# ygtxr1997/MSML

Measured on AMD Instinct MI355X. Metric: images/sec (112x112) ires50-MSML+PartialFC training step, higher is better.
Workload: dtype bf16; 1 GPU; iresnet50-MSML (OSB r18 + FM x4) + 85742-id ArcFace PartialFC, 112x112, batch 256/GPU, fwd+bwd+clip+SGD; global_batch=256, parallelism=dp1+class-parallel head, launch=eager, weight gradients + OSB on side streams

## Files before the change

include/msml_hip.h:

```cpp
#ifndef MSML_HIP_H
#define MSML_HIP_H

#include <stddef.h>
#include <stdint.h>

#ifdef __cplusplus
extern "C" {
#endif

#define MSML_ABI_VERSION 1

enum { MSML_F32 = 0, MSML_BF16 = 1, MSML_BF16X3 = 2 };

enum {
  MSML_OK = 0,
  MSML_ERR_SHAPE = -1,
  MSML_ERR_DTYPE = -2,
  MSML_ERR_LAUNCH = -3,
  MSML_ERR_UNSUPPORTED = -4,
  MSML_ERR_WORKSPACE = -5
};

enum { MSML_ACT_TANH = 0, MSML_ACT_SIGMOID = 1 };
enum { MSML_ARITH_ADD = 0, MSML_ARITH_SUB = 1, MSML_ARITH_MUL = 2, MSML_ARITH_DIV = 3 };
// ... 60 lines not shown
int msml_bn_stats_rows(long M, int C);
int msml_bn_stats(const void* x, long M, int C, float* partial, int dtype, void* stream);
int msml_bn_finalize(const float* partial, int rows, int C, double count, const float* gamma,
                     const float* beta, float* running_mean, float* running_var, float momentum,
                     float eps, float* scale, float* shift, float* save_mean, float* save_invstd,
                     void* stream);
int msml_bn_act_fwd(const void* x, const float* scale, const float* shift, const float* alpha,
                    const void* residual, int res_first, void* y, long M, int C, int dtype,
                    void* stream);
int msml_bn_act_fwd_stats_rows(long M, int C);
int msml_bn_act_fwd_stats(const void* x, const float* scale, const float* shift, const float* alpha,
                          const void* residual, int res_first, void* y, long M, int C,
                          float* stats, int dtype, void* stream);
int msml_bn_fin_act_fwd(const double* acc, double count, const float* gamma, const float* beta,
                        float* running_mean, float* running_var, float momentum, float eps, float* scale,
                        float* shift, float* save_mean, float* save_invstd, const void* x,
                        const float* alpha, const void* residual, int res_first, void* y, long M, int C,
                        double* acc_out, int dtype, void* stream);
int msml_bn_stats_acc(const void* x, long M, int C, double* acc, int dtype, void* stream);
int msml_conv2d_bnbwd_acc(const void* in0, int c0p, const void* wp, int kop, void* out, int coutp, int N,
                          int H, int W, int P, int Q, int R, int S, int stride, int pad_h, int pad_w,
                          int transposed, const void* bn_x, const float* bn_scale, const float* bn_shift,
                          const float* bn_alpha, const float* bn_mean, const float* bn_invstd, double* acc,
                          void* stream);
int msml_bn_fin_bwd_apply(const void* dy, const void* x, const float* scale, const float* shift,
                          const float* alpha, const float* save_mean, const float* save_invstd,
                          const double* acc, const void* residual_first, const void* add, int add_h,
                          int add_w, void* dx, void* dres, float* dgamma, float* dbeta, float* dalpha,
                          int accumulate, long M, int C, const void* next_x, const float* next_mean,
                          const float* next_invstd, double* next_acc, int dtype, void* stream);
int msml_bn_act_bwd_acc(const void* dy, const void* x, const float* scale, const float* shift,
                        const float* alpha, const float* save_mean, const float* save_invstd,
                        const void* residual_first, const void* add, void* dx, void* dres, float* dgamma,
                        float* dbeta, float* dalpha, int accumulate, long M, int C, double* acc, int dtype,
                        void* stream);
int msml_bn_act_bwd(const void* dy, const void* x, const float* scale, const float* shift,
                    const float* alpha, const float* save_mean, const float* save_invstd,
                    const void* residual_first, void* dx, void* dres, float* dgamma, float* dbeta,
                    float* dalpha, int accumulate, long M, int C, float* workspace, long ws_floats,
                    int dtype, void* stream);
int msml_bias_grad(const void* dy, long M, int Cp, int Creal, float* db, int accumulate,
                   float* workspace, long ws_floats, int dtype, void* stream);
int msml_add(const void* a, const void* b, void* out, long n, int dtype, void* stream);

int msml_dap_fwd(const void* x, float* seg, unsigned char* mask, int N, int H, int W, int Cp,
                 int dtype, void* stream);
int msml_dap_bwd(const float* dseg, void* dx, int N, int H, int W, int Cp, int dtype, void* stream);
int msml_seg_consensus_loss(const float* logit, const long* msk, int N, int H, int W, float alpha,
                            float beta, float* loss, float* dlogit, float* workspace,
                            long ws_floats, void* stream);
int msml_seg_consensus_loss_r(const float* logit, const long* msk, int N, int H, int W, float alpha, float beta,
                              int reduce_pixel_all, int reduce_pixel_kl_all, float* loss, float* dlogit,
                              float* workspace, long ws_floats, void* stream);

int msml_rownorm_fwd(const float* w, int R, int Rp, int E, void* dst, int ld, float* inv_norm,
                     int dtype, void* stream);
int msml_rownorm_bwd(const float* w, const float* inv_norm, const float* dy, int ldy, int R, int E,
                     float* dw, int accumulate, void* stream);
int msml_gather_target(const float* cosm, int ld, const long* label, int N, float* out,
                       void* stream);
int msml_margin_fwd(float* cosm, const long* label, int N, int C, int ld, int kind, float s,
                    float m, float a, float k, void* stream);
int msml_margin_bwd(const float* dlogit, int ldg, const long* label, const float* cos_t, int N,
                    int C, void* dcos, int ldo, int kind, float s, float m, float a, float k,
                    int dtype, void* stream);
int msml_pfc_rowstats(const float* cosm, int ld, int N, int C, const long* label, int kind, float s,
                      float m, float a, float k, float* rowmax, float* rowsum, void* stream);
int msml_pfc_grad(const float* cosm, int ld, int N, int C, const long* label, int kind, float s,
                  float m, float a, float k, const float* gmax, const float* gsum, float eps_ls,
                  float inv_n, void* dcos, int ldo, float* ptarget, int dtype, void* stream);
int msml_sgd_momentum(float* w, const float* grad, float* mom, long n, float lr, float mu, float wd,
                      int first_step, const float* clip_coef, void* stream);
int msml_grad_norm_clip(const float* grad, long n, float max_norm, float* out2, float* workspace,
                        long ws_floats, void* stream);
int msml_sgd_momentum_dev(float* w, const float* grad, float* mom, long n, const float* lr, float mu, float wd,
                          const float* coef, void* stream);
int msml_grad_norm_clip_scaled(const float* grad, long n, float max_norm, float scale, float* out2, float* workspace,
                               long ws_floats, void* stream);

long msml_gemm_splitk_workspace(int M, int coutp, int K);
int msml_gemm_splitk(const void* a, int M, int K, const void* wp, int kop, float* out, int coutp,
                     void* workspace, long ws_bytes, int dtype, void* stream);

int msml_pack_weights_batched(const long* table, int count, int dtype, void* stream);
int msml_pack_tiles(int A, int B, int R, int S);
int msml_pack_weights_tiled(const long* table, const int* tile_prefix, int count, int total_tiles,
                            int dtype, void* stream);

int msml_transpose(const void* src, int R, int C, int ld_s, void* dst, int ld_d, int dtype,
                   void* stream);

int msml_conv2d_fused(const void* in0, int c0p, const void* in1, int c1p, const void* wp, int kop,
                      const float* scale, const float* shift, const float* alpha,
                      const void* residual, int res_first, void* out, int coutp, int N, int H,
                      int W, int P, int Q, int R, int S, int stride, int pad_h, int pad_w,
                      int transposed, void* stream);

int msml_conv2d_x3(const void* in0, int c0p, const void* in1, int c1p, const void* wp, int kop,
                   const float* scale, const float* shift, const float* alpha, const void* residual,
                   int res_first, void* out, int coutp, int N, int H, int W, int P, int Q, int R, int S,
                   int stride, int pad_h, int pad_w, int transposed, void* stream);
int msml_conv2d_x3_border(const void* in0, int c0p, const void* wp, int kop, const float* scale,
                          const float* shift9, const float* alpha, const void* residual, int res_first,
                          void* out, int coutp, int N, int H, int W, void* stream);
int msml_x3_bn_act_fwd(const void* x, const float* scale, const float* shift, const float* alpha,
                       const void* residual, int res_first, void* y, long M, int C, void* stream);
int msml_x3_fm_fuse_fwd(const void* x, const void* yf, void* z, long M, int C, int act, int arith,
                        void* stream);
int msml_x3_add(const void* a, const void* b, void* out, long M, int C, void* stream);
int msml_x3_from_f32(const float* src, void* dst, long M, int C, void* stream);
int msml_x3_to_f32(const void* src, float* dst, long M, int C, void* stream);

int msml_pair_sqdist(const float* emb, int n_pairs, int E, double* dist, void* stream);
int msml_pair_sqdist_f64(const double* emb, int n_pairs, int E, double* dist, void* stream);
int msml_pair_hist(const double* dist, const unsigned char* same, int n_pairs, const double* thr, int nthr,
                   int nfolds, int* hist, void* stream);

int msml_occ_draw(long seed, long offset, int N, int H, int W, int mode, int lo, int hi, int flip, int* desc,
                  void* stream);
int msml_occ_apply(const unsigned char* src, const int* desc, float* img, long* msk, float* ori, int N, int H,
                   int W, int light, void* stream);

int msml_occ_draw_tex(long seed, long offset, int N, int H, int W, int mode, int lo, int hi, int flip,
                      const int* meta, int nsets, int* desc, void* stream);
int msml_occ_resize(const unsigned char* atlas, const int* meta, const int* dir, const int* rtab, const int* desc,
                    unsigned char* patch, long patch_stride, int N, int lds_bytes, void* stream);
int msml_occ_apply_tex(const unsigned char* src, const int* desc, const unsigned char* patch, long patch_stride,
                       float* img, long* msk, float* ori, int N, int H, int W, int light, void* stream);

int msml_occ_draw_out(long seed, long offset, int N, int H, int W, int out_h, int out_w, int mode, int lo, int hi,
                      int flip, const int* meta, int nsets, int* desc, void* stream);
int msml_occ_apply_out(const unsigned char* src, const int* desc, const unsigned char* patch, long patch_stride,
                       const int* tabw, const int* tabh, float* img, long* msk, float* ori, int N, int H, int W,
                       int out_h, int out_w, int gray, int norm, int light, void* stream);

int msml_deconv4_bwd_data(const void* dy, const void* wp0, const void* wp1, void* dx0, void* dx1, int N, int H,
                          void* stream);

int msml_conv2d_bnbwd_rows(int coutp, int N, int P, int Q);
int msml_conv2d_bnbwd(const void* in0, int c0p, const void* wp, int kop, void* out, int coutp,
                      int N, int H, int W, int P, int Q, int R, int S, int stride, int pad_h,
                      int pad_w, int transposed, const void* bn_x, const float* bn_scale,
                      const float* bn_shift, const float* bn_alpha, const float* bn_mean,
                      const float* bn_invstd, float* partial, int rows_cap, int* rows_used,
                      void* stream);
int msml_bn_act_bwd_apply(const void* dy, const void* x, const float* scale, const float* shift,
                          const float* alpha, const float* save_mean, const float* save_invstd,
                          const float* partial, int rows, const void* add, void* dx,
                          float* dgamma, float* dbeta, float* dalpha, int accumulate, long M,
                          int C, float* coef_ws, int dtype, void* stream);

int msml_bn_act_bwd_apply_s2(const void* dy, const void* x, const float* scale, const float* shift,
                             const float* alpha, const float* save_mean, const float* save_invstd,
                             const float* partial, int rows, const void* add, int H, int W, void* dx,
                             float* dgamma, float* dbeta, float* dalpha, int accumulate, long M,
                             int C, float* coef_ws, int dtype, void* stream);
int msml_bn_act_bwd_apply_next_s2(const void* dy, const void* x, const float* scale,
                                  const float* shift, const float* alpha, const float* save_mean,
                                  const float* save_invstd, const float* partial, int rows,
                                  const void* add, int H, int W, void* dx, float* dgamma, float* dbeta,
                                  float* dalpha, int accumulate, long M, int C, float* coef_ws,
                                  const void* next_x, const float* next_mean,
                                  const float* next_invstd, float* next_partial, int dtype,
                                  void* stream);

int msml_conv2d_bnin_applies(int c0p, int coutp, int N, int H, int W, int P, int Q, int R, int S,
// ... 80 lines not shown
```

msml_amd/headers/partial_fc.py:

```python
import logging
import os

import torch
import torch.distributed as dist
from torch.nn import Module
from torch.nn.parameter import Parameter


_FORCE = bool(os.environ.get("MSML_FORCE_DIST"))


class _Margin:
    kind = "arc"

    def __init__(self, s=64.0, m=0.5, a=0.0, k=0.0):
        self.s, self.m, self.a, self.k = float(s), float(m), float(a), float(k)

    def __call__(self, logits, labels):
        raise TypeError("msml_amd margins are descriptors consumed by the fused HIP kernels")


class ArcMargin(_Margin):
    kind = "arc"


class CosMargin(_Margin):
    kind = "cos"


class HipBackend:

    def __init__(self, dtype):
        from .. import ops
        from .._lib import TORCH_DTYPE, call
        self.ops, self.call, self.dtype = ops, call, dtype
        self.tdt = TORCH_DTYPE[dtype]

    def local_stats(self, total_features, sub_weight, labels, margin):
        ops, call = self.ops, self.call
        from .. import functional as Fh
        n, e = total_features.shape
        c = sub_weight.shape[0]
        dev = total_features.device
        cp = ops.cpad(c)
        kop = (cp + ops.tile_n(cp) - 1) // ops.tile_n(cp) * ops.tile_n(cp)
        wn = torch.empty(kop, e, dtype=self.tdt, device=dev)
        inv_w = torch.empty(c, dtype=torch.float32, device=dev)
        call("msml_rownorm_fwd", sub_weight.detach(), c, kop, e, wn, e, inv_w, self.dtype)
        xs = total_features.to(self.tdt).reshape(n, 1, 1, e).contiguous()
        cosm, _ = ops.conv2d(xs, None, wn, None, cp, 1, 1, 1, 0, 0, False, out_dtype=0)
        cosm = cosm.reshape(n, cp)
        rowmax = torch.empty(n, dtype=torch.float32, device=dev)
        rowsum = torch.empty(n, dtype=torch.float32, device=dev)
        kind = Fh.HEAD_KIND[margin.kind]
        call("msml_pfc_rowstats", cosm, cp, n, c, labels, kind, margin.s, margin.m, margin.a,
             margin.k, rowmax, rowsum)
        state = (xs, wn, inv_w, cosm, kind)
        return state, rowmax, rowsum

    def local_grads(self, state, sub_weight, labels, margin, gmax, gsum, n_total, eps_ls, dw_out=None):
        ops, call = self.ops, self.call
        xs, wn, inv_w, cosm, kind = state
        n, cp = cosm.shape
        c, e = sub_weight.shape
        dev = cosm.device
        dcos = torch.empty(n, 1, 1, cp, dtype=self.tdt, device=dev)
        ptarget = torch.empty(n, dtype=torch.float32, device=dev)
        call("msml_pfc_grad", cosm, cp, n, c, labels, kind, margin.s, margin.m, margin.a, margin.k,
             gmax, gsum, eps_ls, 1.0 / n_total, dcos, cp, ptarget, self.dtype)
        wnt = torch.empty(e, ops.kpad(cp), dtype=self.tdt, device=dev)
        call("msml_transpose", wn, c, e, e, wnt, ops.kpad(cp), self.dtype)
        if self.dtype == 1:
            dx = ops.gemm_splitk(dcos.reshape(n, cp), wnt, e)
        else:
            dx, _ = ops.conv2d(dcos, None, wnt, None, e, 1, 1, 1, 0, 0, False, out_dtype=0)
        dwn = torch.empty(c, e, dtype=torch.float32, device=dev)
        ops.conv_wgrad(dcos, xs, dwn, c, e, e, 0, 1, 1, 1, 0, 0)
        dw = dw_out if dw_out is not None else torch.empty(c, e, dtype=torch.float32, device=dev)
        call("msml_rownorm_bwd", sub_weight.detach(), inv_w, dwn, e, c, e, dw, 0)
        return ptarget, dx.reshape(n, e), dw


class PartialFC(Module):
    @torch.no_grad()
    def __init__(self, rank, local_rank, world_size, batch_size, resume, margin_softmax, num_classes,
                 sample_rate=1.0, embedding_size=512, prefix="./", fp16=False, backend=None,
                 device=None):
        super().__init__()
        if not isinstance(margin_softmax, _Margin):
            raise TypeError("margin_softmax must be msml_amd.headers.ArcMargin / CosMargin "
                            "(the margin is fused into the HIP softmax kernels)")
        self.num_classes, self.rank, self.local_rank = num_classes, rank, local_rank
        self.device = device if device is not None else torch.device("cuda:{}".format(local_rank))
        self.world_size, self.batch_size = world_size, batch_size
        self.margin_softmax = margin_softmax
        self.sample_rate, self.embedding_size, self.prefix = sample_rate, embedding_size, prefix
        self.num_local = num_classes // world_size + int(rank < num_classes % world_size)
        self.class_start = num_classes // world_size * rank + min(rank, num_classes % world_size)
        self.num_sample = int(self.sample_rate * self.num_local)
        self.weight_name = os.path.join(prefix, "rank:{}_softmax_weight.pt".format(rank))
        self.weight_mom_name = os.path.join(prefix, "rank:{}_softmax_weight_mom.pt".format(rank))
        self.weight = self.weight_mom = None
        if resume:
            try:
                self.weight = torch.load(self.weight_name).to(self.device)
                logging.info("softmax weight resume successfully!")
            except (FileNotFoundError, KeyError, IndexError):
                logging.info("softmax weight resume fail!")
            try:
                self.weight_mom = torch.load(self.weight_mom_name).to(self.device)
                logging.info("softmax weight mom resume successfully!")
            except (FileNotFoundError, KeyError, IndexError):
                logging.info("softmax weight mom resume fail!")
        if self.weight is None:
            self.weight = torch.normal(0, 0.01, (self.num_local, embedding_size), device=self.device)
        if self.weight_mom is None:
            self.weight_mom = torch.zeros_like(self.weight)
        self.stream = torch.cuda.Stream(local_rank) if self.device.type == "cuda" else None
        self.index = None
        self.full = int(self.sample_rate) == 1
        if self.full:
            self.sub_weight = Parameter(self.weight)
            self.sub_weight_mom = self.weight_mom
        else:
            self.sub_weight = Parameter(torch.empty((0, 0), device=self.device))
            self.sub_weight_mom = None
        self._k = None
        self._flat_param = None
        if backend is None:
            from .._lib import BF16, F32
            backend = HipBackend(BF16 if fp16 else F32)
        self.backend = backend
        self.eps_ls = 0.1
        self._stage = None
        self._flat = None
        self._label_job = None
        self.perm_fn = None

    def save_params(self):
        if not self.full and self.index is not None:
            self.update()
        w = self.sub_weight.data if self.full else self.weight
        mom = self.sub_weight_mom if self.full else self.weight_mom
        torch.save(w.detach().clone(), self.weight_name)
        torch.save(mom.detach().clone(), self.weight_mom_name)

    def adopt_flat_optimizer(self, opt):
        if not self.full:
            if self._flat_param is None or self.sub_weight is not self._flat_param or id(self.sub_weight) not in opt.offsets:
                raise ValueError("negative sampling on a flat-arena optimizer: build it over pfc.flat_parameter() "
                                 "(and adopt it before the first prefetch_labels() / forward_backward())")
            if opt.max_norm is not None:
                raise ValueError("the head's FlatSGD must be built with max_norm=None (the reference never clips the "
                                 "PartialFC weight, train.py:267-277)")
            self._flat_mom = opt.momentum_view(self.sub_weight)
            opt.steps = max(opt.steps, 1)
            self._flat = opt
            return
        mview = opt.momentum_view(self.sub_weight)
        mview.copy_(self.weight_mom)
        if self.weight_mom.abs().sum().item() != 0:
            opt.steps = max(opt.steps, 1)
# ... 175 lines not shown
```

msml_amd/csrc/wgrad_halo.hip:

```cpp
#include <stdlib.h>

#include <type_traits>

#include <mutex>

#include "common.h"

typedef __attribute__((ext_vector_type(4))) short s16x4;
typedef __attribute__((ext_vector_type(8))) short s16x8;
typedef __attribute__((address_space(3))) void* lptr_t;

#define WH_OOB 0x78000000u

#define WH_MAXGROUP 8
struct WgradHaloArgs {
  const unsigned short* u[WH_MAXGROUP]; int up; unsigned int u_bytes;
  const unsigned short* v[WH_MAXGROUP]; int vp; unsigned int v_bytes;
  int N, H, W, spy, spx;
  int XH, XW;
  int nstrips, chunk;
  int zper;
  int remap;
  int pair7;
  float* ws;
  BnIn xin;
};

template <int CO, bool XF = false, bool P7 = false>
__global__ void __launch_bounds__(512) __attribute__((amdgpu_waves_per_eu(2, 2))) k_wgrad_halo(const WgradHaloArgs p) {
#if defined(__HIP_DEVICE_COMPILE__)
  constexpr int NXB = 20;
  constexpr int GU = CO / 32, NI = CO / 64, UBLK = 7 * GU, NBLK = UBLK + NXB, NISS = (NBLK + 7) / 8;
  constexpr int UB = UBLK * 1024, VB = NXB * 1024, STAGE = UB + VB;
  extern __shared__ __attribute__((aligned(16))) char smem[];
  MSML_LDS_REGION(smem, 2 * STAGE + (XF ? 3 * 64 * 4 : 0));
  const int t = threadIdx.x, lane = t & 63;
  const int wave = __builtin_amdgcn_readfirstlane(t >> 6);
  const int mp = wave & 1, nh = (wave >> 1) & 1, tg = wave >> 2;
  int bx = blockIdx.x, by = blockIdx.y, bz = blockIdx.z;
  if (p.remap) {
    const int T = gridDim.x * gridDim.y, total = T * gridDim.z;
    const int L = bx + gridDim.x * (by + gridDim.y * bz);
    const int Lp = (L & 7) * (total >> 3) + (L >> 3);
    const int tile = Lp % T;
    bz = Lp / T;
    bx = tile % gridDim.x;
    by = tile / gridDim.x;
  }
  const int layer = __builtin_amdgcn_readfirstlane(bz / p.zper);
  const int a0 = bx * CO, b0 = by * 64, split = bz - layer * p.zper;
  const int s_begin = split * p.chunk;
  int s_end = s_begin + p.chunk;
  if (s_end > p.nstrips) s_end = p.nstrips;
  const int spi = p.spy * p.spx;

  __amdgpu_buffer_rsrc_t rs_u = __builtin_amdgcn_make_buffer_rsrc((void*)p.u[layer], 0, (int)p.u_bytes, 0x00020000);
  __amdgpu_buffer_rsrc_t rs_v = __builtin_amdgcn_make_buffer_rsrc((void*)p.v[layer], 0, (int)p.v_bytes, 0x00020000);

  const int lp = lane >> 2, lc = lane & 3;
  auto issue = [&](int strip, int buf) {
    char* ub = smem + buf * STAGE;
    char* vb = ub + UB;
    if constexpr (P7) {
      const int n = 2 * strip + (lp >> 3), x = lp & 7;
      const bool img = n < p.N;
#pragma unroll
      for (int i = 0; i < NISS; i++) {
        const int blk = wave + 8 * i;
        if (blk >= NBLK) break;
        if (blk < UBLK) {
          const int j = blk / GU, g = blk % GU;
          const unsigned int off = (img & (x < 7)) ? (unsigned int)((n * 7 + j) * 7 + x) * (unsigned int)(p.up * 2) +
                                                         (unsigned int)(a0 + g * 32 + lc * 8) * 2u
                                                   : WH_OOB;
          __builtin_amdgcn_raw_ptr_buffer_load_lds(rs_u, (lptr_t)(ub + blk * 1024), 16, off, 0, 0, 0);
        } else {
          const int bb = blk - UBLK, hr = bb >> 1, g = bb & 1;
          const int y = hr - 1;
          const bool ok = img & ((unsigned)y < 7u) & (x > 0);
          const unsigned int off = ok ? (unsigned int)((n * 7 + y) * 7 + x - 1) * (unsigned int)(p.vp * 2) +
                                            (unsigned int)(b0 + g * 32 + lc * 8) * 2u
                                      : WH_OOB;
          __builtin_amdgcn_raw_ptr_buffer_load_lds(rs_v, (lptr_t)(vb + bb * 1024), 16, off, 0, 0, 0);
        }
      }
      return;
    }
    const int n = strip / spi, rem = strip - n * spi, sy = rem / p.spx;
    const int y0 = sy * 7, x0 = (rem - sy * p.spx) * 14;
#pragma unroll
    for (int i = 0; i < NISS; i++) {
      const int blk = wave + 8 * i;
      if (blk >= NBLK) break;
      if (blk < UBLK) {
        const int j = blk / GU, g = blk % GU;
        const int y = y0 + j, x = x0 + lp;
        const bool ok = (lp < 14) & (x < p.W) & (y < p.H);
        const unsigned int off = ok ? (unsigned int)((n * p.H + y) * p.W + x) * (unsigned int)(p.up * 2) +
                                          (unsigned int)(a0 + g * 32 + lc * 8) * 2u
                                    : WH_OOB;
        __builtin_amdgcn_raw_ptr_buffer_load_lds(rs_u, (lptr_t)(ub + blk * 1024), 16, off, 0, 0, 0);
      } else {
        const int bb = blk - UBLK, hr = bb >> 1, g = bb & 1;
        const int y = y0 + hr - 1, x = x0 + lp - 1;
        const bool ok = (hr < 9) & ((unsigned)y < (unsigned)p.H) & ((unsigned)x < (unsigned)p.W);
        const unsigned int off = ok ? (unsigned int)((n * p.H + y) * p.W + x) * (unsigned int)(p.vp * 2) +
                                          (unsigned int)(b0 + g * 32 + lc * 8) * 2u
                                    : WH_OOB;
        __builtin_amdgcn_raw_ptr_buffer_load_lds(rs_v, (lptr_t)(vb + bb * 1024), 16, off, 0, 0, 0);
      }
    }
  };

  float* xtab = reinterpret_cast<float*>(smem + 2 * STAGE);
  auto xform = [&](int strip, int buf) {
    const int n = strip / spi, rem = strip - n * spi, sy = rem / p.spx;
    const int y0 = sy * 7, x0 = (rem - sy * p.spx) * 14;
    char* vb = smem + buf * STAGE + UB;
    const bool has_alpha = p.xin.alpha != nullptr;
#pragma unroll
    for (int i = 0; i < NISS; i++) {
      const int blk = wave + 8 * i;
      if (blk >= NBLK) break;
      if (blk >= UBLK) {
        const int bb = blk - UBLK, hr = bb >> 1, g = bb & 1;
        const int y = y0 + hr - 1, x = x0 + lp - 1;
        if ((hr < 9) & ((unsigned)y < (unsigned)p.H) & ((unsigned)x < (unsigned)p.W))
          bn_in_chunk(vb + bb * 1024 + lane * 16, xtab, 64, g * 32 + lc * 8, has_alpha);
      }
    }
  };

  f32x16 acc[NI][5];
#pragma unroll
  for (int i = 0; i < NI; i++)
#pragma unroll
    for (int k = 0; k < 5; k++)
#pragma unroll
      for (int e = 0; e < 16; e++) acc[i][k][e] = 0.f;

  const int g4 = lane >> 4, i16 = lane & 15, q4 = i16 >> 2, pp = i16 & 3;
  const int px = 8 * (g4 >> 1) + q4;
  const int chan = (2 * (g4 & 1) + (pp >> 1)) * 16 + (pp & 1) * 8;
  const int aofs = mp * NI * 1024 + px * 64 + chan;
  int vlo[3], vhi[3];
#pragma unroll
  for (int s = 0; s < 3; s++) {
    const int p0 = px + s, p1 = px + 4 + s;
    vlo[s] = nh * 1024 + (p0 >> 4) * 2048 + (p0 & 15) * 64 + chan;
    vhi[s] = nh * 1024 + (p1 >> 4) * 2048 + (p1 & 15) * 64 + chan;
  }
  const int ntaps = tg == 0 ? 5 : 4, tap0 = tg * 5;
  int vlok[5], vhik[5];
#pragma unroll
  for (int k = 0; k < 5; k++) {
    const int tp = tap0 + k, r = tp / 3, sft = tp - r * 3;
    vlok[k] = r * 2048 + (sft == 0 ? vlo[0] : (sft == 1 ? vlo[1] : vlo[2]));
    vhik[k] = r * 2048 + (sft == 0 ? vhi[0] : (sft == 1 ? vhi[1] : vhi[2]));
  }
  typedef __attribute__((address_space(3))) s16x4* tr_ptr;
  auto tr2 = [&](const char* lo, const char* hi) -> s16x8 {
    s16x4 l = __builtin_amdgcn_ds_read_tr16_b64_v4i16((tr_ptr)(lo));
    s16x4 h = __builtin_amdgcn_ds_read_tr16_b64_v4i16((tr_ptr)(hi));
    s16x8 o;
    o[0] = l[0]; o[1] = l[1]; o[2] = l[2]; o[3] = l[3];
    o[4] = h[0]; o[5] = h[1]; o[6] = h[2]; o[7] = h[3];
    return o;
  };

  if (s_begin < s_end) issue(s_begin, 0);
  if (XF) bn_in_fill(p.xin, xtab, b0, 64, t, 512);
  __syncthreads();
  if (XF) {
    if (s_begin < s_end) xform(s_begin, 0);
    __syncthreads();
  }
  int cur = 0;
  s16x8 fa[2][NI], fb5[2][5];
  for (int strip = s_begin; strip < s_end; strip++) {
    if (strip + 1 < s_end) issue(strip + 1, cur ^ 1);
    const char* ub = smem + cur * STAGE + aofs;
    const char* vb = smem + cur * STAGE + UB;
    auto fetch = [&](int j, int fb) {
#pragma unroll
      for (int i = 0; i < NI; i++)
        fa[fb][i] = tr2(ub + j * (GU * 1024) + i * 1024, ub + j * (GU * 1024) + i * 1024 + 256);
#pragma unroll
      for (int k = 0; k < 5; k++)
        if (k < ntaps) fb5[fb][k] = tr2(vb + j * 2048 + vlok[k], vb + j * 2048 + vhik[k]);
    };
    fetch(0, 0);
#pragma unroll
    for (int j = 0; j < 7; j++) {
      const int fb = j & 1;
      if (j + 1 < 7) fetch(j + 1, fb ^ 1);
      __builtin_amdgcn_sched_barrier(0);
#pragma unroll
      for (int k = 0; k < 5; k++)
        if (k < ntaps) {
#pragma unroll
          for (int i = 0; i < NI; i++)
            acc[i][k] = __builtin_amdgcn_mfma_f32_32x32x16_bf16(__builtin_bit_cast(bf16x8, fa[fb][i]),
                                                                __builtin_bit_cast(bf16x8, fb5[fb][k]), acc[i][k], 0, 0, 0);
        }
      __builtin_amdgcn_sched_barrier(0);
      if (XF && j == (CO == 128 ? 6 : 2) && strip + 1 < s_end) {
        asm volatile("s_waitcnt vmcnt(0)" ::: "memory");
        xform(strip + 1, cur ^ 1);
      }
    }
    __syncthreads();
    cur ^= 1;
  }

  const int h = lane >> 5, c32 = lane & 31;
  const int b = b0 + nh * 32 + c32;
#pragma unroll
  for (int i = 0; i < NI; i++)
#pragma unroll
    for (int k = 0; k < 5; k++) {
      if (k >= ntaps) continue;
#pragma unroll
      for (int e = 0; e < 16; e++) {
        const int a = a0 + (mp * NI + i) * 32 + (e & 3) + 8 * (e >> 2) + 4 * h;
        p.ws[(((long)bz * p.up + a) * 9 + tap0 + k) * p.vp + b] = acc[i][k][e];
      }
    }
#endif
}

static int wh_cus() {
  static int n = 0;
  if (n == 0) {
    int dev = 0;
    if (hipGetDevice(&dev) != hipSuccess || hipDeviceGetAttribute(&n, hipDeviceAttributeMultiprocessorCount, dev) != hipSuccess || n <= 0)
      n = 256;
  }
  return n;
}

static bool wh_wide(int up) {
  static const int lim = getenv("MSML_WGRAD_HALO_WIDE_MIN") ? atoi(getenv("MSML_WGRAD_HALO_WIDE_MIN")) : 128;
  return up % 128 == 0 && up >= lim;
}

int msml_wgrad_halo_splits(int up, int vp, int A, int Breal, int N, int H, int W, int P, int Q, int R, int S,
                           int stride, int pad_h, int pad_w) {
  static const bool off = getenv("MSML_NO_HALO_WGRAD") != nullptr;
  if (off) return 0;
  if (R != 3 || S != 3 || stride != 1 || pad_h != 1 || pad_w != 1 || P != H || Q != W) return 0;
  if (up % 64 != 0 || vp % 64 != 0 || A != up || Breal != vp) return 0;
  const bool pair7 = H == 7 && W == 7 && getenv("MSML_WGRAD_HALO_NO_PAIR7") == nullptr;
  const long strips = pair7 ? (N + 1) / 2 : (long)N * cdiv(H, 7) * cdiv(W, 14);
  if ((long)N * H * W * 10 < strips * 112 * 7) return 0;
  if ((long)N * H * W * up * 2 >= 0x70000000L || (long)N * H * W * vp * 2 >= 0x70000000L) return 0;
  const int tiles = ((wh_wide(up) && !pair7) ? up / 128 : up / 64) * (vp / 64);
  long splits = wh_cus() / tiles;
  if (splits < 1) splits = 1;
  if (splits > strips) splits = strips;
  if (splits > 512) splits = 512;
  return (int)splits;
}

template <int CO, bool XF, bool P7 = false>
static void wh_launch(const WgradHaloArgs& a, dim3 grid, hipStream_t st) {
  const size_t lds = 2 * (7 * (CO / 32) + 10 * 2) * 1024 + (XF ? 3 * 64 * sizeof(float) : 0);
  static std::once_flag attr_once;
  std::call_once(attr_once, [&] {
    (void)hipFuncSetAttribute(reinterpret_cast<const void*>(&k_wgrad_halo<CO, XF, P7>),
                              hipFuncAttributeMaxDynamicSharedMemorySize, (int)lds);
  });
  k_wgrad_halo<CO, XF, P7><<<grid, dim3(512), lds, st>>>(a);
}

int msml_wgrad_halo_group_splits(int up, int vp, int A, int Breal, int N, int H, int W, int P, int Q, int R, int S,
                                 int stride, int pad_h, int pad_w, int group) {
  const int hs = msml_wgrad_halo_splits(up, vp, A, Breal, N, H, W, P, Q, R, S, stride, pad_h, pad_w);
  if (hs <= 0 || group < 1 || group > WH_MAXGROUP) return 0;
  const int per = hs / group;
  return per < 1 ? 0 : per;
}

bool msml_wgrad_halo_launch_group(const void* const* u, int up, const void* const* v, int vp, float* ws, int N, int H,
                                  int W, int group, int splits, hipStream_t st, const BnIn* xin) {
  static const bool no_remap = getenv("MSML_WGRAD_HALO_NO_REMAP") != nullptr;
  WgradHaloArgs a;
  for (int i = 0; i < WH_MAXGROUP; i++) {
    a.u[i] = (const unsigned short*)u[i < group ? i : 0];
    a.v[i] = (const unsigned short*)v[i < group ? i : 0];
  }
  a.up = up; a.u_bytes = (unsigned int)((long)N * H * W * up * 2);
  a.vp = vp; a.v_bytes = (unsigned int)((long)N * H * W * vp * 2);
  a.N = N; a.H = H; a.W = W; a.spy = cdiv(H, 7); a.spx = cdiv(W, 14);
  a.pair7 = (H == 7 && W == 7) ? 1 : 0;
  a.nstrips = a.pair7 ? (N + 1) / 2 : N * a.spy * a.spx;
  a.chunk = cdiv(a.nstrips, splits);
  a.zper = splits;
  a.ws = ws;
  a.xin = BnIn{nullptr, nullptr, nullptr};
  if (xin) a.xin = *xin;
  const int gz = group * splits;
  const int tiles = ((wh_wide(up) && !a.pair7) ? up / 128 : up / 64) * (vp / 64);
  a.remap = (!no_remap && tiles >= 4 && gz % 8 == 0) ? 1 : 0;
  if (a.pair7) {
    if (xin) return false;
    wh_launch<64, false, true>(a, dim3(up / 64, vp / 64, gz), st);
    return true;
// ... 16 lines not shown
```

Baseline: 8901 images/sec.

## Add fused PartialFC backward kernels for dx and rownorm-fused dW

Adds two HIP kernels for the PartialFC head backward in bf16 with E=512. The dx kernel is a split-K MFMA GEMM that reads the normalized weight directly, which removes the transpose copy of wn, and it folds partial sums through a workspace. The dW kernel computes dcos^T·x with MFMA and applies the row-norm backward in its epilogue, so the fp32 dwn intermediate is never written and no separate rownorm_bwd pass runs. The Python side tries the fused kernels first and falls back to the old path on error. The costs are added kernel complexity and an extra fold pass when dx is split over K.

After: 8959 images/sec (median of 6 runs). About the same (+0.6%).

```diff
diff --git a/include/msml_hip.h b/include/msml_hip.h
--- a/include/msml_hip.h
+++ b/include/msml_hip.h
@@ -166,6 +166,13 @@
 int msml_gemm_splitk(const void* a, int M, int K, const void* wp, int kop, float* out, int coutp,
                      void* workspace, long ws_bytes, int dtype, void* stream);
 
+int msml_pfc_dw(const void* dcos, int ldc, const void* x, int ldx, const float* w, const float* inv_norm, int N, int C,
+                int E, float* dw, int dtype, void* stream);
+
+long msml_pfc_dx_workspace(int N, int C, int E);
+int msml_pfc_dx(const void* dcos, int ldc, const void* wn, int wn_rows, int N, int C, int E, float* out,
+                void* workspace, long ws_bytes, int dtype, void* stream);
+
 int msml_pack_weights_batched(const long* table, int count, int dtype, void* stream);
 int msml_pack_tiles(int A, int B, int R, int S);
 int msml_pack_weights_tiled(const long* table, const int* tile_prefix, int count, int total_tiles,
diff --git a/msml_amd/csrc/pfc_fused.hip b/msml_amd/csrc/pfc_fused.hip
--- /dev/null
+++ b/msml_amd/csrc/pfc_fused.hip
@@ -0,0 +1,349 @@
+#include <stdlib.h>
+
+#include <mutex>
+
+#include "common.h"
+
+typedef __attribute__((ext_vector_type(4))) short s16x4;
+typedef __attribute__((ext_vector_type(8))) short s16x8;
+typedef __attribute__((address_space(3))) void* lptr_t;
+
+#define PFC_OOB 0x7ffffff0u
+#define PDW_E 512
+#define PDW_BLOCKS 36
+#define PDW_STAGE (PDW_BLOCKS * 1024)
+#define PDW_LDS (2 * PDW_STAGE)
+
+struct PfcDwArgs {
+  const unsigned short* dcos; unsigned int dcos_bytes; int ldc;
+  const unsigned short* x; unsigned int x_bytes; int ldx;
+  const float* w; const float* inv_w; float* dw;
+  int N, C;
+};
+
+__global__ void __launch_bounds__(256, 2) k_pfc_dw(const PfcDwArgs p) {
+#if defined(__HIP_DEVICE_COMPILE__)
+  extern __shared__ __attribute__((aligned(16))) char smem[];
+  MSML_LDS_REGION(smem, PDW_LDS);
+  const int t = threadIdx.x, lane = t & 63;
+  const int wave = __builtin_amdgcn_readfirstlane(t >> 6);
+  const int c0 = blockIdx.x * 64;
+  const int nstages = (p.N + 31) >> 5;
+
+  __amdgpu_buffer_rsrc_t rs_u = __builtin_amdgcn_make_buffer_rsrc((void*)p.dcos, 0, (int)p.dcos_bytes, 0x00020000);
+  __amdgpu_buffer_rsrc_t rs_v = __builtin_amdgcn_make_buffer_rsrc((void*)p.x, 0, (int)p.x_bytes, 0x00020000);
+
+  const int lp = lane >> 2, lc = lane & 3;
+  auto issue = [&](int stage, int buf) {
+    char* sb = smem + buf * PDW_STAGE;
+#pragma unroll
+    for (int i = 0; i < PDW_BLOCKS / 4; i++) {
+      const int blk = wave + 4 * i;
+      const int kk = blk >= 18 ? 1 : 0, r = blk - 18 * kk;
+      const int n = stage * 32 + kk * 16 + lp;
+      const bool nok = n < p.N;
+      if (r < 2) {
+        const int col = c0 + r * 32 + lc * 8;
+        const unsigned int off = (nok && col < p.ldc) ? ((unsigned int)n * (unsigned int)p.ldc + (unsigned int)col) * 2u : PFC_OOB;
+        __builtin_amdgcn_raw_ptr_buffer_load_lds(rs_u, (lptr_t)(sb + blk * 1024), 16, off, 0, 0, 0);
+      } else {
+        const int col = (r - 2) * 32 + lc * 8;
+        const unsigned int off = nok ? ((unsigned int)n * (unsigned int)p.ldx + (unsigned int)col) * 2u : PFC_OOB;
+        __builtin_amdgcn_raw_ptr_buffer_load_lds(rs_v, (lptr_t)(sb + blk * 1024), 16, off, 0, 0, 0);
+      }
+    }
+  };
+
+  f32x16 acc[2][4];
+#pragma unroll
+  for (int i = 0; i < 2; i++)
+#pragma unroll
+    for (int j = 0; j < 4; j++)
+#pragma unroll
+      for (int e = 0; e < 16; e++) acc[i][j][e] = 0.f;
+
+  const int g4 = lane >> 4, i16 = lane & 15, q4 = i16 >> 2, pp = i16 & 3;
+  const int frag = (8 * (g4 >> 1) + q4) * 64 + (2 * (g4 & 1) + (pp >> 1)) * 16 + (pp & 1) * 8;
+  typedef __attribute__((address_space(3))) s16x4* tr_ptr;
+  auto tr2 = [&](const char* lo) -> s16x8 {
+    s16x4 l = __builtin_amdgcn_ds_read_tr16_b64_v4i16((tr_ptr)(lo));
+    s16x4 h = __builtin_amdgcn_ds_read_tr16_b64_v4i16((tr_ptr)(lo + 256));
+    s16x8 o;
+    o[0] = l[0]; o[1] = l[1]; o[2] = l[2]; o[3] = l[3];
+    o[4] = h[0]; o[5] = h[1]; o[6] = h[2]; o[7] = h[3];
+    return o;
+  };
+
+  issue(0, 0);
+  int cur = 0;
+  for (int st = 0; st < nstages; st++) {
+    asm volatile("s_waitcnt vmcnt(0)" ::: "memory");
+    __syncthreads();
+    if (st + 1 < nstages) issue(st + 1, cur ^ 1);
+#pragma unroll
+    for (int kk = 0; kk < 2; kk++) {
+      const char* sb = smem + cur * PDW_STAGE + kk * (18 * 1024) + frag;
+      s16x8 a[2], b[4];
+#pragma unroll
+      for (int i = 0; i < 2; i++) a[i] = tr2(sb + i * 1024);
+#pragma unroll
+      for (int j = 0; j < 4; j++) b[j] = tr2(sb + (2 + wave * 4 + j) * 1024);
+#pragma unroll
+      for (int i = 0; i < 2; i++)
+#pragma unroll
+        for (int j = 0; j < 4; j++)
+          acc[i][j] = __builtin_amdgcn_mfma_f32_32x32x16_bf16(__builtin_bit_cast(bf16x8, a[i]), __builtin_bit_cast(bf16x8, b[j]),
+                                                           acc[i][j], 0, 0, 0);
+    }
+    cur ^= 1;
+  }
+  __syncthreads();
+
+  float* tile = reinterpret_cast<float*>(smem);
+  MSML_LDS_REGION(tile, 32 * PDW_E * 4);
+  const int h = lane >> 5, c32 = lane & 31;
+#pragma unroll
+  for (int hf = 0; hf < 2; hf++) {
+#pragma unroll
+    for (int j = 0; j < 4; j++)
+#pragma unroll
+      for (int e = 0; e < 16; e++)
+        tile[((e & 3) + 8 * (e >> 2) + 4 * h) * PDW_E + wave * 128 + j * 32 + c32] = acc[hf][j][e];
+    __syncthreads();
+#pragma unroll 4
+    for (int it = 0; it < 8; it++) {
+      const int r = wave * 8 + it;
+      const int c = c0 + 32 * hf + r;
+      if (c < p.C) {
+        const float inv = p.inv_w[c];
+        const float* wr = p.w + (long)c * PDW_E + lane * 4;
+        const float* gr = tile + r * PDW_E + lane * 4;
+        f32x4 pv[2], gv[2];
+        float dot = 0.f;
+#pragma unroll
+        for (int k = 0; k < 2; k++) {
+          pv[k] = *reinterpret_cast<const f32x4*>(wr + k * 256);
+          gv[k] = *reinterpret_cast<const f32x4*>(gr + k * 256);
+#pragma unroll
+          for (int j = 0; j < 4; j++) dot += pv[k][j] * inv * gv[k][j];
+        }
+        dot = wave_sum(dot);
+        float* o = p.dw + (long)c * PDW_E + lane * 4;
+#pragma unroll
+        for (int k = 0; k < 2; k++) {
+          f32x4 v;
+#pragma unroll
+          for (int j = 0; j < 4; j++) v[j] = (gv[k][j] - pv[k][j] * inv * dot) * inv;
+          *reinterpret_cast<f32x4*>(o + k * 256) = v;
+        }
+      }
+    }
+    __syncthreads();
+  }
+#endif
+}
+
+static bool pfc_fused_off() {
+  static const bool off = getenv("MSML_NO_PFC_FUSED") != nullptr;
+  return off;
+}
+
+extern "C" int msml_pfc_dw(const void* dcos, int ldc, const void* x, int ldx, const float* w, const float* inv_norm,
+                           int N, int C, int E, float* dw, int dtype, void* stream) {
+  MSML_CHECK(dcos && x && w && inv_norm && dw && N > 0 && C > 0 && E > 0 && ldc >= C && ldx >= E, MSML_ERR_SHAPE,
+             "pfc_dw: bad args N=%d C=%d E=%d ldc=%d ldx=%d", N, C, E, ldc, ldx);
+  MSML_CHECK(!pfc_fused_off(), MSML_ERR_UNSUPPORTED, "pfc_dw: switched off (MSML_NO_PFC_FUSED)");
+  MSML_CHECK(dtype == MSML_BF16 && E == PDW_E, MSML_ERR_UNSUPPORTED, "pfc_dw: bf16 operands and E = 512 only");
+  MSML_CHECK(ldc % 8 == 0 && ldx % 8 == 0 && ((size_t)dcos % 16) == 0 && ((size_t)x % 16) == 0 && ((size_t)w % 16) == 0 &&
+                 ((size_t)dw % 16) == 0,
+             MSML_ERR_UNSUPPORTED, "pfc_dw: operands must be 16-byte aligned with row strides that are multiples of 8");
+  const long ub = (long)N * ldc * 2, vb = (long)N * ldx * 2;
+  MSML_CHECK(ub < 0x7fffff00L && vb < 0x7fffff00L, MSML_ERR_UNSUPPORTED, "pfc_dw: operands too large for 32-bit offsets");
+  PfcDwArgs a;
+  a.dcos = (const unsigned short*)dcos; a.dcos_bytes = (unsigned int)ub; a.ldc = ldc;
+  a.x = (const unsigned short*)x; a.x_bytes = (unsigned int)vb; a.ldx = ldx;
+  a.w = w; a.inv_w = inv_norm; a.dw = dw;
+  a.N = N; a.C = C;
+  static std::once_flag once;
+  std::call_once(once, [] {
+    (void)hipFuncSetAttribute(reinterpret_cast<const void*>(&k_pfc_dw), hipFuncAttributeMaxDynamicSharedMemorySize, PDW_LDS);
+  });
+  k_pfc_dw<<<cdiv(C, 64), 256, PDW_LDS, (hipStream_t)stream>>>(a);
+  MSML_LAUNCH_OK("pfc_dw");
+  return MSML_OK;
+}
+
+#define PDX_NISS 12
+#define PDX_STAGE (48 * 1024)
+#define PDX_LDS (3 * PDX_STAGE)
+
+struct PfcDxArgs {
+  const unsigned short* dcos; unsigned int dcos_bytes; int ldc;
+  const unsigned short* wn; unsigned int wn_bytes; int wn_rows;
+  int N, E, K, ks, chunk;
+  float* ws;
+};
+
+__global__ void __launch_bounds__(256) k_pfc_dx(const PfcDxArgs p) {
+#if defined(__HIP_DEVICE_COMPILE__)
+  extern __shared__ __attribute__((aligned(16))) char smem[];
+  MSML_LDS_REGION(smem, PDX_LDS);
+  const int t = threadIdx.x, lane = t & 63;
+  const int wave = __builtin_amdgcn_readfirstlane(t >> 6);
+  const int chunk_id = blockIdx.x % p.ks, e0 = (blockIdx.x / p.ks) * 128, m0 = blockIdx.y * 256;
+  const int kb = chunk_id * p.chunk;
+  int ke = kb + p.chunk;
+  if (ke > p.K) ke = p.K;
+  const int nstages = ke > kb ? (ke - kb + 63) >> 6 : 0;
+
+  __amdgpu_buffer_rsrc_t rs_a = __builtin_amdgcn_make_buffer_rsrc((void*)p.dcos, 0, (int)p.dcos_bytes, 0x00020000);
+  __amdgpu_buffer_rsrc_t rs_b = __builtin_amdgcn_make_buffer_rsrc((void*)p.wn, 0, (int)p.wn_bytes, 0x00020000);
+
+  const int lp = lane >> 2, lc = lane & 3;
+  const int ar = lane & 31, ak = (lane >> 5) * 8;
+  auto issue = [&](int stage, int buf) {
+    char* sb = smem + buf * PDX_STAGE;
+    const int k0 = kb + stage * 64;
+#pragma unroll
+    for (int i = 0; i < PDX_NISS; i++) {
+      const int blk = wave + 4 * i;
+      if (blk < 32) {
+        const int row = m0 + (blk & 7) * 32 + ar, col = k0 + (blk >> 3) * 16 + ak;
+        const unsigned int off = (row < p.N && col < ke) ? ((unsigned int)row * (unsigned int)p.ldc + (unsigned int)col) * 2u : PFC_OOB;
+        __builtin_amdgcn_raw_ptr_buffer_load_lds(rs_a, (lptr_t)(sb + blk * 1024), 16, off, 0, 0, 0);
+      } else {
+        const int b = blk - 32;
+        const int k = k0 + (b >> 2) * 16 + lp, col = e0 + (b & 3) * 32 + lc * 8;
+        const unsigned int off = (k < ke && k < p.wn_rows) ? ((unsigned int)k * (unsigned int)p.E + (unsigned int)col) * 2u : PFC_OOB;
+        __builtin_amdgcn_raw_ptr_buffer_load_lds(rs_b, (lptr_t)(sb + blk * 1024), 16, off, 0, 0, 0);
+      }
+    }
+  };
+
+  f32x16 acc[2][4];
+#pragma unroll
+  for (int i = 0; i < 2; i++)
+#pragma unroll
+    for (int j = 0; j < 4; j++)
+#pragma unroll
+      for (int e = 0; e < 16; e++) acc[i][j][e] = 0.f;
+
+  const int g4 = lane >> 4, i16 = lane & 15, q4 = i16 >> 2, pp = i16 & 3;
+  const int frag = (8 * (g4 >> 1) + q4) * 64 + (2 * (g4 & 1) + (pp >> 1)) * 16 + (pp & 1) * 8;
+  typedef __attribute__((address_space(3))) s16x4* tr_ptr;
+  auto tr2 = [&](const char* lo) -> s16x8 {
+    s16x4 l = __builtin_amdgcn_ds_read_tr16_b64_v4i16((tr_ptr)(lo));
+    s16x4 h = __builtin_amdgcn_ds_read_tr16_b64_v4i16((tr_ptr)(lo + 256));
+    s16x8 o;
+    o[0] = l[0]; o[1] = l[1]; o[2] = l[2]; o[3] = l[3];
+    o[4] = h[0]; o[5] = h[1]; o[6] = h[2]; o[7] = h[3];
+    return o;
+  };
+
+  if (nstages > 0) issue(0, 0);
+  if (nstages > 1) issue(1, 1);
+  int cur = 0, nxt = 2;
+  for (int st = 0; st < nstages; st++) {
+    if (st + 1 < nstages) asm volatile("s_waitcnt vmcnt(%0)" ::"n"(PDX_NISS) : "memory");
+    else asm volatile("s_waitcnt vmcnt(0)" ::: "memory");
+    __builtin_amdgcn_s_barrier();
+    if (st + 2 < nstages) issue(st + 2, nxt);
+    const char* sb = smem + cur * PDX_STAGE;
+#pragma unroll
+    for (int k16 = 0; k16 < 4; k16++) {
+      s16x8 a[2], b[4];
+#pragma unroll
+      for (int i = 0; i < 2; i++)
+        a[i] = *reinterpret_cast<const s16x8*>(sb + (k16 * 8 + wave * 2 + i) * 1024 + lane * 16);
+#pragma unroll
+      for (int j = 0; j < 4; j++) b[j] = tr2(sb + (32 + k16 * 4 + j) * 1024 + frag);
+#pragma unroll
+      for (int i = 0; i < 2; i++)
+#pragma unroll
+        for (int j = 0; j < 4; j++)
+          acc[i][j] = __builtin_amdgcn_mfma_f32_32x32x16_bf16(__builtin_bit_cast(bf16x8, a[i]), __builtin_bit_cast(bf16x8, b[j]),
+                                                           acc[i][j], 0, 0, 0);
+    }
+    cur = cur == 2 ? 0 : cur + 1;
+    nxt = nxt == 2 ? 0 : nxt + 1;
+  }
+
+  const int h = lane >> 5, c32 = lane & 31;
+  float* slab = p.ws + (long)chunk_id * p.N * p.E;
+#pragma unroll
+  for (int i = 0; i < 2; i++)
+#pragma unroll
+    for (int e = 0; e < 16; e++) {
+      const int m = m0 + wave * 64 + i * 32 + (e & 3) + 8 * (e >> 2) + 4 * h;
+      if (m < p.N) {
+#pragma unroll
+        for (int j = 0; j < 4; j++) slab[(long)m * p.E + e0 + j * 32 + c32] = acc[i][j][e];
+      }
+    }
+#endif
+}
+
+__global__ void __launch_bounds__(256) k_pfc_dx_fold(const float* __restrict__ ws, float* __restrict__ out, long n4, int ks) {
+  const long i = blockIdx.x * 256L + threadIdx.x;
+  if (i >= n4) return;
+  const f32x4* s = reinterpret_cast<const f32x4*>(ws) + i;
+  f32x4 v = s[0];
+  for (int k = 1; k < ks; k++) {
+    const f32x4 u = s[(long)k * n4];
+    v[0] += u[0]; v[1] += u[1]; v[2] += u[2]; v[3] += u[3];
+  }
+  reinterpret_cast<f32x4*>(out)[i] = v;
+}
+
+static void pfc_dx_split(int N, int C, int E, int* ks, int* chunk) {
+  const int tiles = cdiv(N, 256) * (E / 128);
+  int want = cdiv(256, tiles);
+  want = (want + 7) / 8 * 8;
+  const int stages = cdiv(C, 64);
+  if (want > stages) want = stages;
+  const int per = cdiv(stages, want);
+  *chunk = per * 64;
+  *ks = cdiv(stages, per);
+}
+
+extern "C" long msml_pfc_dx_workspace(int N, int C, int E) {
+  if (N <= 0 || C <= 0 || E != PDW_E) return 0;
+  int ks, chunk;
+  pfc_dx_split(N, C, E, &ks, &chunk);
+  return ks > 1 ? (long)ks * N * E * (long)sizeof(float) : 0;
+}
+
+extern "C" int msml_pfc_dx(const void* dcos, int ldc, const void* wn, int wn_rows, int N, int C, int E, float* out,
+                           void* workspace, long ws_bytes, int dtype, void* stream) {
+  MSML_CHECK(dcos && wn && out && N > 0 && C > 0 && E > 0 && ldc >= C && wn_rows >= C, MSML_ERR_SHAPE,
+             "pfc_dx: bad args N=%d C=%d E=%d ldc=%d wn_rows=%d", N, C, E, ldc, wn_rows);
+  MSML_CHECK(!pfc_fused_off(), MSML_ERR_UNSUPPORTED, "pfc_dx: switched off (MSML_NO_PFC_FUSED)");
+  MSML_CHECK(dtype == MSML_BF16 && E == PDW_E, MSML_ERR_UNSUPPORTED, "pfc_dx: bf16 operands and E = 512 only");
+  MSML_CHECK(ldc % 8 == 0 && ((size_t)dcos % 16) == 0 && ((size_t)wn % 16) == 0 && ((size_t)out % 16) == 0 &&
+                 ((size_t)workspace % 16) == 0,
+             MSML_ERR_UNSUPPORTED, "pfc_dx: operands must be 16-byte aligned, ldc a multiple of 8");
+  const long ab = (long)N * ldc * 2, bb = (long)wn_rows * E * 2;
+  MSML_CHECK(ab < 0x7fffff00L && bb < 0x7fffff00L, MSML_ERR_UNSUPPORTED, "pfc_dx: operands too large for 32-bit offsets");
+  const long need = msml_pfc_dx_workspace(N, C, E);
+  MSML_CHECK(ws_bytes >= need && (need == 0 || workspace), MSML_ERR_WORKSPACE, "pfc_dx: workspace %ld < %ld bytes", ws_bytes, need);
+  PfcDxArgs a;
+  pfc_dx_split(N, C, E, &a.ks, &a.chunk);
+  a.dcos = (const unsigned short*)dcos; a.dcos_bytes = (unsigned int)ab; a.ldc = ldc;
+  a.wn = (const unsigned short*)wn; a.wn_bytes = (unsigned int)bb; a.wn_rows = wn_rows;
+  a.N = N; a.E = E; a.K = (C + 7) / 8 * 8;
+  if (a.K > ldc) a.K = ldc;
+  a.ws = a.ks > 1 ? (float*)workspace : out;
+  static std::once_flag once;
+  std::call_once(once, [] {
+    (void)hipFuncSetAttribute(reinterpret_cast<const void*>(&k_pfc_dx), hipFuncAttributeMaxDynamicSharedMemorySize, PDX_LDS);
+  });
+  hipStream_t st = (hipStream_t)stream;
+  k_pfc_dx<<<dim3(a.ks * (E / 128), cdiv(N, 256)), 256, PDX_LDS, st>>>(a);
+  MSML_LAUNCH_OK("pfc_dx");
+  if (a.ks > 1) {
+    const long n4 = (long)N * E / 4;
+    k_pfc_dx_fold<<<cdiv(n4, 256), 256, 0, st>>>(a.ws, out, n4, a.ks);
+    MSML_LAUNCH_OK("pfc_dx_fold");
+  }
+  return MSML_OK;
+}
diff --git a/msml_amd/headers/partial_fc.py b/msml_amd/headers/partial_fc.py
--- a/msml_amd/headers/partial_fc.py
+++ b/msml_amd/headers/partial_fc.py
@@ -32,8 +32,9 @@
 
     def __init__(self, dtype):
         from .. import ops
-        from .._lib import TORCH_DTYPE, call
-        self.ops, self.call, self.dtype = ops, call, dtype
+        from .._lib import TORCH_DTYPE, call, try_call, value
+        self.ops, self.call, self.try_call, self.value, self.dtype = ops, call, try_call, value, dtype
+        self._dx_ws = {}
         self.tdt = TORCH_DTYPE[dtype]
 
     def local_stats(self, total_features, sub_weight, labels, margin):
@@ -68,16 +69,34 @@
         ptarget = torch.empty(n, dtype=torch.float32, device=dev)
         call("msml_pfc_grad", cosm, cp, n, c, labels, kind, margin.s, margin.m, margin.a, margin.k,
              gmax, gsum, eps_ls, 1.0 / n_total, dcos, cp, ptarget, self.dtype)
-        wnt = torch.empty(e, ops.kpad(cp), dtype=self.tdt, device=dev)
-        call("msml_transpose", wn, c, e, e, wnt, ops.kpad(cp), self.dtype)
+        dx = None
         if self.dtype == 1:
-            dx = ops.gemm_splitk(dcos.reshape(n, cp), wnt, e)
-        else:
-            dx, _ = ops.conv2d(dcos, None, wnt, None, e, 1, 1, 1, 0, 0, False, out_dtype=0)
-        dwn = torch.empty(c, e, dtype=torch.float32, device=dev)
-        ops.conv_wgrad(dcos, xs, dwn, c, e, e, 0, 1, 1, 1, 0, 0)
+            need = self._dx_ws.get((n, c, e))
+            if need is None:
+                need = self._dx_ws[(n, c, e)] = self.value("msml_pfc_dx_workspace", n, c, e)
+            ws = ops.workspace(need, dev)
+            dx = torch.empty(n, e, dtype=torch.float32, device=dev)
+            with ops.PROFILE.rec("pfc_dx", 2.0 * n * c * e):
+                rc = self.try_call("msml_pfc_dx", dcos, cp, wn, wn.shape[0], n, c, e, dx, ws, ws.numel(), self.dtype)
+            if rc != 0:
+                dx = None
+        if dx is None:
+            wnt = torch.empty(e, ops.kpad(cp), dtype=self.tdt, device=dev)
+            call("msml_transpose", wn, c, e, e, wnt, ops.kpad(cp), self.dtype)
+            if self.dtype == 1:
+                dx = ops.gemm_splitk(dcos.reshape(n, cp), wnt, e)
+            else:
+                dx, _ = ops.conv2d(dcos, None, wnt, None, e, 1, 1, 1, 0, 0, False, out_dtype=0)
         dw = dw_out if dw_out is not None else torch.empty(c, e, dtype=torch.float32, device=dev)
-        call("msml_rownorm_bwd", sub_weight.detach(), inv_w, dwn, e, c, e, dw, 0)
+        fused = False
+        if self.dtype == 1:
+            with ops.PROFILE.rec("pfc_dw", 2.0 * n * c * e):
+                fused = self.try_call("msml_pfc_dw", dcos, cp, xs, e, sub_weight.detach(), inv_w, n, c, e, dw,
+                                      self.dtype) == 0
+        if not fused:
+            dwn = torch.empty(c, e, dtype=torch.float32, device=dev)
+            ops.conv_wgrad(dcos, xs, dwn, c, e, e, 0, 1, 1, 1, 0, 0)
+            call("msml_rownorm_bwd", sub_weight.detach(), inv_w, dwn, e, c, e, dw, 0)
         return ptarget, dx.reshape(n, e), dw
 
 
```

## Remap CO=128 wgrad halo waves to 4x2 tiles with rolling row-register reuse

Applied to the files above, without the earlier changes.

For the CO=128 variant, each wave now owns one 32-row A tile and all 9 taps instead of splitting taps across wave groups. It keeps a rolling 4-row register window of shifted V fragments, so each input row is read from LDS once and reused across three filter rows, which cuts LDS transpose reads. The LDS DMA loads switch from the compiler builtin to inline asm that sets m0 by hand, with explicit vmcnt waits before barriers. The cost is more accumulator registers (9 f32x16 per wave) and hand-managed asm that could be fragile.

After: 8701 images/sec before, 8870 images/sec after (median of 6 runs). 1.02x the previous value.

```diff
diff --git a/msml_amd/csrc/wgrad_halo.hip b/msml_amd/csrc/wgrad_halo.hip
--- a/msml_amd/csrc/wgrad_halo.hip
+++ b/msml_amd/csrc/wgrad_halo.hip
@@ -11,6 +11,22 @@
 typedef __attribute__((address_space(3))) void* lptr_t;
 
 #define WH_OOB 0x78000000u
+
+typedef __attribute__((ext_vector_type(4))) unsigned int wh_rsrc_t;
+__device__ __forceinline__ void wh_dma16(const wh_rsrc_t& rs, unsigned int lds, unsigned int off) {
+#if defined(__HIP_DEVICE_COMPILE__)
+  unsigned int keep;
+  asm volatile("s_mov_b32 %0, m0\n\ts_mov_b32 m0, %3\n\ts_nop 0\n\tbuffer_load_dwordx4 %1, %2, 0 offen lds\n\ts_mov_b32 m0, %0"
+               : "=&s"(keep)
+               : "v"(off), "s"(rs), "s"(lds)
+               : "memory");
+#endif
+}
+__device__ __forceinline__ void wh_dma_wait() {
+#if defined(__HIP_DEVICE_COMPILE__)
+  asm volatile("s_waitcnt vmcnt(0)" ::: "memory");
+#endif
+}
 
 #define WH_MAXGROUP 8
 struct WgradHaloArgs {
@@ -36,7 +52,8 @@
   MSML_LDS_REGION(smem, 2 * STAGE + (XF ? 3 * 64 * 4 : 0));
   const int t = threadIdx.x, lane = t & 63;
   const int wave = __builtin_amdgcn_readfirstlane(t >> 6);
-  const int mp = wave & 1, nh = (wave >> 1) & 1, tg = wave >> 2;
+  constexpr bool R9 = CO == 128;
+  const int mp = R9 ? (wave & 3) : (wave & 1), nh = R9 ? (wave >> 2) : ((wave >> 1) & 1), tg = R9 ? 0 : (wave >> 2);
   int bx = blockIdx.x, by = blockIdx.y, bz = blockIdx.z;
   if (p.remap) {
     const int T = gridDim.x * gridDim.y, total = T * gridDim.z;
@@ -54,8 +71,20 @@
   if (s_end > p.nstrips) s_end = p.nstrips;
   const int spi = p.spy * p.spx;
 
-  __amdgpu_buffer_rsrc_t rs_u = __builtin_amdgcn_make_buffer_rsrc((void*)p.u[layer], 0, (int)p.u_bytes, 0x00020000);
-  __amdgpu_buffer_rsrc_t rs_v = __builtin_amdgcn_make_buffer_rsrc((void*)p.v[layer], 0, (int)p.v_bytes, 0x00020000);
+  auto make_rsrc = [](const void* ptr, unsigned int bytes) -> wh_rsrc_t {
+    const unsigned long long a = (unsigned long long)ptr;
+    wh_rsrc_t r;
+    r[0] = __builtin_amdgcn_readfirstlane((unsigned int)a);
+    r[1] = __builtin_amdgcn_readfirstlane((unsigned int)(a >> 32) & 0xffffu);
+    r[2] = __builtin_amdgcn_readfirstlane(bytes);
+    r[3] = 0x00020000u;
+    return r;
+  };
+  const wh_rsrc_t rs_u = make_rsrc(p.u[layer], p.u_bytes), rs_v = make_rsrc(p.v[layer], p.v_bytes);
+  const unsigned int lds0 = __builtin_amdgcn_readfirstlane((unsigned int)(size_t)(lptr_t)smem);
+  auto dma = [&](const wh_rsrc_t& rs, const char* dst, unsigned int off) {
+    wh_dma16(rs, lds0 + (unsigned int)__builtin_amdgcn_readfirstlane((int)(dst - smem)), off);
+  };
 
   const int lp = lane >> 2, lc = lane & 3;
   auto issue = [&](int strip, int buf) {
@@ -73,7 +102,7 @@
           const unsigned int off = (img & (x < 7)) ? (unsigned int)((n * 7 + j) * 7 + x) * (unsigned int)(p.up * 2) +
                                                          (unsigned int)(a0 + g * 32 + lc * 8) * 2u
                                                    : WH_OOB;
-          __builtin_amdgcn_raw_ptr_buffer_load_lds(rs_u, (lptr_t)(ub + blk * 1024), 16, off, 0, 0, 0);
+          dma(rs_u, ub + blk * 1024, off);
         } else {
           const int bb = blk - UBLK, hr = bb >> 1, g = bb & 1;
           const int y = hr - 1;
@@ -81,7 +110,7 @@
           const unsigned int off = ok ? (unsigned int)((n * 7 + y) * 7 + x - 1) * (unsigned int)(p.vp * 2) +
                                             (unsigned int)(b0 + g * 32 + lc * 8) * 2u
                                       : WH_OOB;
-          __builtin_amdgcn_raw_ptr_buffer_load_lds(rs_v, (lptr_t)(vb + bb * 1024), 16, off, 0, 0, 0);
+          dma(rs_v, vb + bb * 1024, off);
         }
       }
       return;
@@ -99,7 +128,7 @@
         const unsigned int off = ok ? (unsigned int)((n * p.H + y) * p.W + x) * (unsigned int)(p.up * 2) +
                                           (unsigned int)(a0 + g * 32 + lc * 8) * 2u
                                     : WH_OOB;
-        __builtin_amdgcn_raw_ptr_buffer_load_lds(rs_u, (lptr_t)(ub + blk * 1024), 16, off, 0, 0, 0);
+        dma(rs_u, ub + blk * 1024, off);
       } else {
         const int bb = blk - UBLK, hr = bb >> 1, g = bb & 1;
         const int y = y0 + hr - 1, x = x0 + lp - 1;
@@ -107,7 +136,7 @@
         const unsigned int off = ok ? (unsigned int)((n * p.H + y) * p.W + x) * (unsigned int)(p.vp * 2) +
                                           (unsigned int)(b0 + g * 32 + lc * 8) * 2u
                                     : WH_OOB;
-        __builtin_amdgcn_raw_ptr_buffer_load_lds(rs_v, (lptr_t)(vb + bb * 1024), 16, off, 0, 0, 0);
+        dma(rs_v, vb + bb * 1024, off);
       }
     }
   };
@@ -131,18 +160,19 @@
     }
   };
 
-  f32x16 acc[NI][5];
-#pragma unroll
-  for (int i = 0; i < NI; i++)
-#pragma unroll
-    for (int k = 0; k < 5; k++)
+  constexpr int NA = R9 ? 1 : NI, NK = R9 ? 9 : 5;
+  f32x16 acc[NA][NK];
+#pragma unroll
+  for (int i = 0; i < NA; i++)
+#pragma unroll
+    for (int k = 0; k < NK; k++)
 #pragma unroll
       for (int e = 0; e < 16; e++) acc[i][k][e] = 0.f;
 
   const int g4 = lane >> 4, i16 = lane & 15, q4 = i16 >> 2, pp = i16 & 3;
   const int px = 8 * (g4 >> 1) + q4;
   const int chan = (2 * (g4 & 1) + (pp >> 1)) * 16 + (pp & 1) * 8;
-  const int aofs = mp * NI * 1024 + px * 64 + chan;
+  const int aofs = mp * NA * 1024 + px * 64 + chan;
   int vlo[3], vhi[3];
 #pragma unroll
   for (int s = 0; s < 3; s++) {
@@ -150,7 +180,7 @@
     vlo[s] = nh * 1024 + (p0 >> 4) * 2048 + (p0 & 15) * 64 + chan;
     vhi[s] = nh * 1024 + (p1 >> 4) * 2048 + (p1 & 15) * 64 + chan;
   }
-  const int ntaps = tg == 0 ? 5 : 4, tap0 = tg * 5;
+  const int ntaps = R9 ? 9 : (tg == 0 ? 5 : 4), tap0 = tg * 5;
   int vlok[5], vhik[5];
 #pragma unroll
   for (int k = 0; k < 5; k++) {
@@ -170,20 +200,54 @@
 
   if (s_begin < s_end) issue(s_begin, 0);
   if (XF) bn_in_fill(p.xin, xtab, b0, 64, t, 512);
+  wh_dma_wait();
   __syncthreads();
   if (XF) {
     if (s_begin < s_end) xform(s_begin, 0);
     __syncthreads();
   }
   int cur = 0;
-  s16x8 fa[2][NI], fb5[2][5];
+  s16x8 fa[2][NA], fb5[2][5], xr[4][3];
   for (int strip = s_begin; strip < s_end; strip++) {
     if (strip + 1 < s_end) issue(strip + 1, cur ^ 1);
     const char* ub = smem + cur * STAGE + aofs;
     const char* vb = smem + cur * STAGE + UB;
+    if constexpr (R9) {
+      auto fetch_a = [&](int j) { fa[j & 1][0] = tr2(ub + j * (GU * 1024), ub + j * (GU * 1024) + 256); };
+      auto fetch_x = [&](int row) {
+#pragma unroll
+        for (int sft = 0; sft < 3; sft++) xr[row & 3][sft] = tr2(vb + row * 2048 + vlo[sft], vb + row * 2048 + vhi[sft]);
+      };
+      fetch_a(0);
+      fetch_x(0);
+      fetch_x(1);
+      fetch_x(2);
+#pragma unroll
+      for (int j = 0; j < 7; j++) {
+        if (j + 1 < 7) {
+          fetch_a(j + 1);
+          fetch_x(j + 3);
+        }
+        __builtin_amdgcn_sched_barrier(0);
+#pragma unroll
+        for (int k = 0; k < 9; k++)
+          acc[0][k] = __builtin_amdgcn_mfma_f32_32x32x16_bf16(__builtin_bit_cast(bf16x8, fa[j & 1][0]),
+                                                              __builtin_bit_cast(bf16x8, xr[(j + k / 3) & 3][k % 3]),
+                                                              acc[0][k], 0, 0, 0);
+        __builtin_amdgcn_sched_barrier(0);
+        if (XF && j == 6 && strip + 1 < s_end) {
+          wh_dma_wait();
+          xform(strip + 1, cur ^ 1);
+        }
+      }
+      wh_dma_wait();
+      __syncthreads();
+      cur ^= 1;
+      continue;
+    }
     auto fetch = [&](int j, int fb) {
 #pragma unroll
-      for (int i = 0; i < NI; i++)
+      for (int i = 0; i < NA; i++)
         fa[fb][i] = tr2(ub + j * (GU * 1024) + i * 1024, ub + j * (GU * 1024) + i * 1024 + 256);
 #pragma unroll
       for (int k = 0; k < 5; k++)
@@ -199,7 +263,7 @@
       for (int k = 0; k < 5; k++)
         if (k < ntaps) {
 #pragma unroll
-          for (int i = 0; i < NI; i++)
+          for (int i = 0; i < NA; i++)
             acc[i][k] = __builtin_amdgcn_mfma_f32_32x32x16_bf16(__builtin_bit_cast(bf16x8, fa[fb][i]),
                                                                 __builtin_bit_cast(bf16x8, fb5[fb][k]), acc[i][k], 0, 0, 0);
         }
@@ -209,6 +273,7 @@
         xform(strip + 1, cur ^ 1);
       }
     }
+    wh_dma_wait();
     __syncthreads();
     cur ^= 1;
   }
@@ -216,13 +281,13 @@
   const int h = lane >> 5, c32 = lane & 31;
   const int b = b0 + nh * 32 + c32;
 #pragma unroll
-  for (int i = 0; i < NI; i++)
-#pragma unroll
-    for (int k = 0; k < 5; k++) {
+  for (int i = 0; i < NA; i++)
+#pragma unroll
+    for (int k = 0; k < NK; k++) {
       if (k >= ntaps) continue;
 #pragma unroll
       for (int e = 0; e < 16; e++) {
-        const int a = a0 + (mp * NI + i) * 32 + (e & 3) + 8 * (e >> 2) + 4 * h;
+        const int a = a0 + (mp * NA + i) * 32 + (e & 3) + 8 * (e >> 2) + 4 * h;
         p.ws[(((long)bz * p.up + a) * 9 + tap0 + k) * p.vp + b] = acc[i][k][e];
       }
     }
```
